# gkm2708/gym-lmaze

Measured on AMD Instinct MI355X. Metric: env steps/sec (whole node), 1M parallel 11x11 mazes at 1/2/4/8 MI355X, higher is better.
Workload: dtype int32

## Files before the change

gym-lmaze_amd/csrc/lmaze_step.hip:

```cpp
#include <cstdio>

#include <cmath>
#include <cstdlib>

#include "lmaze_common.h"
#include "lmaze_policy_table.h"

namespace lmaze {

static constexpr size_t kNonTemporalObsBytes = (size_t)192 << 20;

template <bool NT, int BITS = 0>
__device__ __forceinline__ void store16(int4* p, const int4& v) {
    typedef int v4i __attribute__((ext_vector_type(4)));
    if (NT) {
        v4i t = {v.x, v.y, v.z, v.w};
        stream_store16<BITS>(reinterpret_cast<v4i*>(p), t);
    } else {
        *p = v;
    }
}

__device__ __forceinline__ void count_goal(int32_t* p) { __hip_atomic_fetch_add(p, 1, __ATOMIC_RELAXED, __HIP_MEMORY_SCOPE_AGENT); }

__host__ __device__ inline bool beyond_caches(int64_t n, int cells) { return (size_t)n * cells * 4 > kNonTemporalObsBytes; }

struct EnvState {
    int2 b, g;
    int act, sc, done;
    float r;
};

template <int VARIANT, bool DO_STEP>
__device__ __forceinline__ EnvState load_env(const StepArgs& a, int64_t e) {
    constexpr bool V3 = VARIANT == LMAZE_VARIANT_V3;
    EnvState in;
    in.b = a.ball[e];
    in.g = make_int2(-1, -1);
    if (V3) in.g = a.goal[e];
    in.act = 0; in.sc = 0; in.done = 0; in.r = 0.0f;
    if (DO_STEP) {
        in.act = a.action[e];
        in.sc = a.step_count[e];
        if (!V3) in.r = a.reward[e];
        const uint8_t* dp = a.auto_reset ? a.done + e : a.layout;
        in.done = *dp;
    }
    return in;
}

template <int VARIANT>
__device__ __forceinline__ void env_reset(int ball_cell, int goal_cell, int G, EnvState& s) {
    if (ball_cell >= 0) s.b = make_int2(ball_cell / G, ball_cell % G);
    if (VARIANT == LMAZE_VARIANT_V3 && goal_cell >= 0) s.g = make_int2(goal_cell / G, goal_cell % G);
    s.sc = 0;
    s.r = -0.0f;
}

__device__ __forceinline__ void clamp_ball(EnvState& s, int G) { s.b = make_int2(clampi(s.b.x, 0, G - 1), clampi(s.b.y, 0, G - 1)); }

template <int VARIANT, class CellAt>
__device__ __forceinline__ bool env_advance(const StepArgs& a, int G, CellAt cell_at, EnvState& s) {
    int bx = clampi(s.b.x, 0, G - 1), by = clampi(s.b.y, 0, G - 1);
    s.sc += 1;
    int ox, oy;
    decode_action(s.act, ox, oy);
    const int tx = clampi(bx + ox, 0, G - 1), ty = clampi(by + oy, 0, G - 1);
    float r;
    bool dn;
    const bool hit = transition_rule<VARIANT>(a, cell_at(tx, ty), ox, oy, tx, ty, s.sc, s.r, s.g.x, s.g.y, bx, by, r, dn);
    s.b = make_int2(bx, by);
    s.r = r;
    s.done = dn ? 1 : 0;
    return hit;
}

__device__ __forceinline__ void store_state(const StepArgs& a, int64_t e, const EnvState& s) {
    a.ball[e] = s.b;
    a.step_count[e] = s.sc;
    a.reward[e] = s.r;
    a.done[e] = s.done;
}

__device__ __forceinline__ int ball_cell_of(const int2& b, int G) { return b.x * G + b.y; }
template <int VARIANT>
__device__ __forceinline__ int goal_cell_of(const int2& g, int G) {
// ... 427 lines not shown
                a.step_count[e] = sc;
                a.reward[e] = r;
                a.done[e] = dn ? 1 : 0;
            }
            b = make_int2(bx, by);
        } else {
            b = make_int2(clampi(b.x, 0, G - 1), clampi(b.y, 0, G - 1));
        }
        if (a.obs == nullptr) continue;
        const int bcell = b.x * G + b.y;
        const int gcell = (V3 && g.x >= 0 && g.x < G && g.y >= 0 && g.y < G) ? g.x * G + g.y : -8;
        int4* obs4 = reinterpret_cast<int4*>(a.obs + (size_t)e * CELLS);
#pragma unroll
        for (int j = 0; j < NJ; ++j) {
            const int c0 = (j * 64 + lane) << 2;
            int vals[4];
#pragma unroll
            for (int q = 0; q < 4; ++q) {
                int v = cell_bits<VARIANT>((uint8_t)(w[j] >> (8 * q)));
                v |= (bcell == c0 + q) ? LMAZE_OBS_BALL : 0;
                if (V3) v |= (gcell == c0 + q) ? LMAZE_OBS_GOAL : 0;
                vals[q] = v;
            }
            store16<NT, 2>(obs4 + j * 64 + lane, make_int4(vals[0], vals[1], vals[2], vals[3]));
        }
    }
}


template <int VARIANT, bool DO_STEP, int EPW>
__global__ __launch_bounds__(LMAZE_BLOCK) void step_shared_wave8_kernel(const StepArgs a) {
    constexpr bool V3 = VARIANT == LMAZE_VARIANT_V3;
    constexpr int G = 8, CELLS = 64;
    const int lane = threadIdx.x & 63;
    const int64_t base = ((int64_t)blockIdx.x * (blockDim.x >> 6) + (threadIdx.x >> 6)) * EPW;
    if (base >= a.n) return;
    const int nb = (int)min((int64_t)EPW, a.n - base);
    const bool autoreset = DO_STEP && a.auto_reset;
    const uint64_t epoch = step_epoch(a, autoreset);
    const bool live = lane < nb;
    const int myc = a.layout[lane];
    EnvState s{};
    s.b = make_int2(1, 1); s.g = make_int2(-1, -1);
    if (live) s = load_env<VARIANT, DO_STEP>(a, base + lane);
    const int mypat = cell_bits<VARIANT>((uint8_t)myc);
    const int p4 = (lane & 15) << 2;
    const int4 pat4 = make_int4(__shfl(mypat, p4, 64), __shfl(mypat, p4 + 1, 64), __shfl(mypat, p4 + 2, 64),
                                __shfl(mypat, p4 + 3, 64));
    int4* obs4 = reinterpret_cast<int4*>(a.obs + (size_t)base * CELLS);
    if (DO_STEP) {
        if (autoreset) {
            const unsigned long long ok[1] = {__ballot(interior(lane, G) && spawn_ok<VARIANT>((uint8_t)myc))};
            if (s.done) {
                int bc, gc;
                place_from_masks<VARIANT, 1>(ok, __popcll(ok[0]), env_draw(a.seed, epoch, a.env_base + base + lane), bc, gc);
                env_reset<VARIANT>(bc, gc, G, s);
                if (V3 && gc >= 0 && live) a.goal_rw[base + lane] = s.g;
            }
        }
        const bool hit = env_advance<VARIANT>(a, G, [&](int tx, int ty) { return (uint8_t)__shfl(myc, tx * G + ty, 64); }, s);
        if (live) {
            const int64_t e = base + lane;
            if (hit && a.goal_count) count_goal(a.goal_count + e);
            store_state(a, e, s);
        }
    } else {
        clamp_ball(s, G);
    }
    if (a.obs == nullptr) return;
    const int ball_cell = ball_cell_of(s.b, G);
    const int goal_cell = goal_cell_of<VARIANT>(s.g, G);
#pragma unroll
    for (int k = 0; k < EPW / 4; ++k) {
        const int le = (lane >> 4) + 4 * k;
        const int bc = __shfl(ball_cell, le, 64);
        const int gc = V3 ? __shfl(goal_cell, le, 64) : -8;
        int4 v = pat4;
        or_at(v, bc - p4, LMAZE_OBS_BALL);
        if (V3) or_at(v, gc - p4, LMAZE_OBS_GOAL);
        if (le < nb) obs4[lane + 64 * k] = v;
    }
}

template <int VARIANT, bool DO_STEP, int EPB>
__global__ __launch_bounds__(LMAZE_BLOCK) void step_shared_u8_kernel(const StepArgs a) {
    constexpr bool V3 = VARIANT == LMAZE_VARIANT_V3;
    static_assert(EPB % 16 == 0 && EPB <= LMAZE_BLOCK, "a workgroup's byte range starts on a 16-byte boundary; one lane per env");
    const int G = a.grid, CELLS = G * G;
    const int PW = (2 * CELLS + 16 + 3) >> 2;
    extern __shared__ int4 lds4[];
    uint32_t* patw = reinterpret_cast<uint32_t*>(lds4);
    int* ballflat = reinterpret_cast<int*>(patw + 4 * PW);
    int* goalflat = ballflat + EPB + 1;
    int* maskflag = goalflat + EPB + 1;
    uint16_t* spawn = reinterpret_cast<uint16_t*>(maskflag + EPB + 1);
    uint8_t* lay = reinterpret_cast<uint8_t*>(spawn + ((CELLS + 1) & ~1));
    __shared__ int spawn_count_s;
    const int tid = threadIdx.x;
    const int64_t nchunks = (a.n + EPB - 1) / EPB;
    int64_t chunk = blockIdx.x;
    int64_t blockbase = chunk * EPB;
    int nb = (int)min((int64_t)EPB, a.n - blockbase);
    const bool masked = !DO_STEP && a.mask != nullptr;
    const bool autoreset = DO_STEP && a.auto_reset;
    const uint64_t epoch = step_epoch(a, autoreset);
    EnvState in{};
    if (tid < nb) in = load_env<VARIANT, DO_STEP>(a, blockbase + tid);
    int warmed = 0;
    if (DO_STEP && (a.launch_hint & 0x100)) {
        warmed = warm_lines(a.action, a.n * 4, 256) + warm_lines(a.ball, a.n * 8, 256) + warm_lines(a.step_count, a.n * 4, 256);
        if (!V3) warmed += warm_lines(a.reward, a.n * 4, 256);
        if (V3) warmed += warm_lines(a.goal, a.n * 8, 256);
        if (autoreset) warmed += warm_lines(a.done, a.n, 256);
    }
    for (int i = tid; i < CELLS; i += LMAZE_BLOCK) lay[i] = a.layout[i];
    __syncthreads();
    uint8_t* patb = reinterpret_cast<uint8_t*>(patw);
    for (int i = tid; i < 4 * PW; i += LMAZE_BLOCK) {
        const int s = i / PW, k = (i - s * PW) << 2;
        uint32_t w = 0;
#pragma unroll
        for (int j = 0; j < 4; ++j) {
            int c = k + s + j;
            c -= c >= CELLS ? CELLS : 0;
            c -= c >= CELLS ? CELLS : 0;
            c = min(c, CELLS - 1);
            w |= (uint32_t)cell_bits<VARIANT>(lay[c]) << (8 * j);
        }
        patw[i] = w;
    }
    if (autoreset && tid < 64) {
        const int cnt = wave_build_spawn_list<VARIANT>(lay, G, CELLS, spawn, tid);
        if (tid == 0) spawn_count_s = cnt;
    }
    if (tid == 0) { ballflat[EPB] = -64; goalflat[EPB] = -64; maskflag[EPB] = 0; }
    __syncthreads();
  for (;;) {
    const int64_t next = chunk + gridDim.x;
    const bool has_next = next < nchunks;
    EnvState in_next{};
    int nb_next = 0;
    if (has_next) {
        nb_next = (int)min((int64_t)EPB, a.n - next * EPB);
        if (tid < nb_next) in_next = load_env<VARIANT, DO_STEP>(a, next * EPB + tid);
    }
    if (tid < EPB) {
        int bf = -64, gf = -64, mf = 0;
        if (tid < nb) {
            const int64_t e = blockbase + tid;
            int bc, gc;
            const int cnt = autoreset ? spawn_count_s : 0;
            env_phase1<VARIANT, DO_STEP>(a, lay, G, e, in, [&](uint4 d, int& pb, int& pg) { place_from_list<VARIANT>(spawn, cnt, d, pb, pg); }, epoch, bc, gc);
            bf = bc;
            if (V3 && gc >= 0) gf = gc;
            if (masked) mf = a.mask[e] != 0;
        }
        ballflat[tid] = bf;
        goalflat[tid] = gf;
        maskflag[tid] = mf;
    }
    if (a.obs8 != nullptr) {
    __syncthreads();
    uint8_t* obs = a.obs8 + (size_t)blockbase * CELLS;
    const int R = nb * CELLS;
    if (!masked) {
        const int nq = R >> 4;
        for (int q = tid; q < nq; q += LMAZE_BLOCK) {
// ... 528 lines not shown
    if (layout_mode != LMAZE_LAYOUT_SHARED) return launch_perenv<GT, VARIANT, DO_STEP>(a, s);
    if constexpr (GT == 8) {
        const bool small = a.obs == nullptr || !beyond_caches(a.n, 64);
        if (small && a.mask == nullptr && (a.launch_hint & 0x100) == 0) {
            int code = (a.launch_hint >> 4) & 15;
            if (code < 1 || code > 3) code = a.n >= 65536 ? 1 : 2;
            const int epw = 128 >> code;
            int wpb = a.launch_hint & 15;
            if (wpb != 1 && wpb != 2 && wpb != 4) wpb = a.n >= 65536 ? 4 : 1;
            const int64_t waves = (a.n + epw - 1) / epw;
            const int64_t blocks = (waves + wpb - 1) / wpb;
            if (!grid_ok(blocks)) return hipErrorInvalidConfiguration;
            const dim3 grid((unsigned)blocks), block(64 * wpb);
            if (a.info) {
                char name[96];
                snprintf(name, sizeof(name), "step_shared_wave8_kernel<v%d, %s, %d>", VARIANT, DO_STEP ? "step" : "observe", epw);
                describe_launch(a.info, name, epw * wpb, 0, 1, false, blocks, 64 * wpb, 0);
                return hipSuccess;
            }
            if (code == 1) hipLaunchKernelGGL((step_shared_wave8_kernel<VARIANT, DO_STEP, 64>), grid, block, 0, s, a);
            else if (code == 2) hipLaunchKernelGGL((step_shared_wave8_kernel<VARIANT, DO_STEP, 32>), grid, block, 0, s, a);
            else hipLaunchKernelGGL((step_shared_wave8_kernel<VARIANT, DO_STEP, 16>), grid, block, 0, s, a);
            return hipGetLastError();
        }
        int sel = (a.launch_hint >> 10) & 3;
        if (sel == 0) sel = table_sel<VARIANT>(a, a.obs != nullptr ? 2 : 1);
        if (sel == 2) return launch_shared<GT, VARIANT, DO_STEP, 64>(a, s);
        return launch_shared<GT, VARIANT, DO_STEP, 128>(a, s);
    } else if constexpr (GT == 11 || GT == 12) {
        int sel = (a.launch_hint >> 10) & 3;
        const bool streaming = a.obs != nullptr && beyond_caches(a.n, GT * GT);
        if (sel == 0) {
            if (GT == 11) sel = streaming ? 2 : 1;
            else sel = streaming ? 3 : 1;
            if (streaming) sel = table_sel<VARIANT>(a, sel);
        }
        if (sel == 2) return launch_shared<GT, VARIANT, DO_STEP, 32>(a, s);
        if (sel == 3) return launch_shared<GT, VARIANT, DO_STEP, 16>(a, s);
        return launch_shared<GT, VARIANT, DO_STEP, 64>(a, s);
    } else if constexpr (GT == 14 || GT == 18) {
        int sel = (a.launch_hint >> 10) & 3;
        const bool streaming = a.obs != nullptr && beyond_caches(a.n, GT * GT);
        if (sel == 0) sel = ((GT == 14 || VARIANT == LMAZE_VARIANT_V3) && streaming) ? 2 : 1;
        if (((a.launch_hint >> 10) & 3) == 0 && streaming) sel = table_sel<VARIANT>(a, sel);
        if (sel == 2) return launch_shared<GT, VARIANT, DO_STEP, 16>(a, s);
        return launch_shared<GT, VARIANT, DO_STEP, 32>(a, s);
    } else if constexpr (GT == 32) {
        int sel = (a.launch_hint >> 10) & 3;
        const bool streaming = a.obs != nullptr && beyond_caches(a.n, GT * GT);
        if (sel == 0) sel = streaming ? table_sel<VARIANT>(a, 2) : 1;
        if (sel == 2) return launch_shared<GT, VARIANT, DO_STEP, 4>(a, s);
        return launch_shared<GT, VARIANT, DO_STEP, 8>(a, s);
    } else {
        int sel = (a.launch_hint >> 10) & 3;
        if (sel == 0) {
            sel = a.grid >= 15 ? 3 : (a.grid >= 5 ? 2 : 1);
            if (a.obs != nullptr && beyond_caches(a.n, a.grid * a.grid) && a.grid >= 5) sel = table_sel<VARIANT>(a, sel);
        }
        if (sel == 3) return launch_shared<GT, VARIANT, DO_STEP, 16>(a, s);
        if (sel == 2) return launch_shared<GT, VARIANT, DO_STEP, 64>(a, s);
        return launch_shared<GT, VARIANT, DO_STEP, 256>(a, s);
    }
}

template <int VARIANT, bool DO_STEP>
static hipError_t dispatch_grid(const StepArgs& a, int layout_mode, hipStream_t s) {
    switch (a.grid) {
        case 8:  return launch_one<8, VARIANT, DO_STEP>(a, layout_mode, s);
        case 11: return launch_one<11, VARIANT, DO_STEP>(a, layout_mode, s);
        case 12: return launch_one<12, VARIANT, DO_STEP>(a, layout_mode, s);
        case 14: return launch_one<14, VARIANT, DO_STEP>(a, layout_mode, s);
        case 18: return launch_one<18, VARIANT, DO_STEP>(a, layout_mode, s);
        case 32: return launch_one<32, VARIANT, DO_STEP>(a, layout_mode, s);
        default: return launch_one<0, VARIANT, DO_STEP>(a, layout_mode, s);
    }
}

hipError_t launch_step(int variant, bool do_step, const StepArgs& a, int layout_mode, hipStream_t s);

#ifndef LMAZE_U8_DEFAULT_SEL
#define LMAZE_U8_DEFAULT_SEL 1
#endif
#ifndef LMAZE_U8_DEFAULT_CHUNKS
#define LMAZE_U8_DEFAULT_CHUNKS 2
#endif
template <int EPB>
static hipError_t launch_step_u8_epb(int variant, bool do_step, const StepArgs& a, hipStream_t s) {
    const int cells = a.grid * a.grid, pw = (2 * cells + 16 + 3) >> 2;
    const size_t lds = ((size_t)4 * pw * 4 + 3 * (size_t)(EPB + 1) * 4 + (size_t)((cells + 1) & ~1) * 2 + (size_t)cells + 15) & ~(size_t)15;
    int m = (a.launch_hint >> 4) & 15;
    if (m == 0) m = LMAZE_U8_DEFAULT_CHUNKS;
    const int64_t nchunks = (a.n + EPB - 1) / EPB;
    const int64_t blocks = (nchunks + m - 1) / m;
    if (!grid_ok(blocks)) return hipErrorInvalidConfiguration;
    if (a.info) {
        char name[96];
        snprintf(name, sizeof(name), "step_shared_u8_kernel<v%d, %s, %d>", variant, do_step ? "step" : "observe", EPB);
        describe_launch(a.info, name, EPB, 0, m, false, blocks, LMAZE_BLOCK, lds);
        return hipSuccess;
    }
    const dim3 grid((unsigned)blocks), block(LMAZE_BLOCK);
    StepArgs b = a;
    b.launch_hint = (a.launch_hint & ~0x100) | ((size_t)a.n * cells > ((size_t)64 << 20) ? 0x100 : 0);
    if (variant == LMAZE_VARIANT_V3) {
        if (do_step) hipLaunchKernelGGL((step_shared_u8_kernel<LMAZE_VARIANT_V3, true, EPB>), grid, block, lds, s, b);
        else hipLaunchKernelGGL((step_shared_u8_kernel<LMAZE_VARIANT_V3, false, EPB>), grid, block, lds, s, b);
    } else {
        if (do_step) hipLaunchKernelGGL((step_shared_u8_kernel<LMAZE_VARIANT_V0, true, EPB>), grid, block, lds, s, b);
        else hipLaunchKernelGGL((step_shared_u8_kernel<LMAZE_VARIANT_V0, false, EPB>), grid, block, lds, s, b);
    }
    return hipGetLastError();
}

hipError_t launch_step_u8(int variant, bool do_step, const StepArgs& a, hipStream_t s) {
    if (a.n == 0) return hipSuccess;
    int sel = (a.launch_hint >> 10) & 3;
    if (sel == 0) sel = LMAZE_U8_DEFAULT_SEL;
    if (sel == 1) return launch_step_u8_epb<256>(variant, do_step, a, s);
    if (sel == 2) return launch_step_u8_epb<128>(variant, do_step, a, s);
    return launch_step_u8_epb<64>(variant, do_step, a, s);
}

static bool slot_stores_nt(const StepArgs& a, const RolloutRec* rec) {
    return rec && rec->obs_t && ((a.launch_hint >> 15) & 1);
}

enum RolloutFamily { RO_WAVE8, RO_SHARED, RO_PERENV, RO_U8, RO_STEPS };
static const char* const kRolloutKernel[] = {"rollout_shared_wave8_kernel", "rollout_shared_kernel", "rollout_perenv_kernel",
                                             "rollout_shared_u8_kernel"};
struct RolloutPlan {
    RolloutFamily family;
    int epb;
    int block;
    int64_t blocks;
    size_t lds;
    bool nt;
};

static size_t rollout_u8_lds_bytes(int G, int epb) {
    const int cells = G * G, pw = (2 * cells + 16 + 3) >> 2;
    return ((size_t)4 * pw * 4 + 2 * (size_t)(epb + 1) * 4 + (size_t)((cells + 1) & ~1) * 2 + (size_t)cells + 15) & ~(size_t)15;
}

static size_t policy_table_lds_bytes(int G) { return (size_t)((G * G + 15) & ~15); }

enum { PLAN_OPEN = 0, PLAN_POLICY = 1, PLAN_SAMPLE_LDS = 2, PLAN_SAMPLE_GLOBAL = 3 };
static RolloutPlan rollout_plan(const StepArgs& a, int layout_mode, int32_t T, const RolloutRec* rec, bool u8, int pol = PLAN_OPEN) {
    const int cells = a.grid * a.grid;
    const bool sample = pol == PLAN_SAMPLE_LDS || pol == PLAN_SAMPLE_GLOBAL;
    const size_t tab = pol == PLAN_POLICY ? policy_table_lds_bytes(a.grid) : pol == PLAN_SAMPLE_LDS ? (size_t)16 * cells : 0;
    const int hint_epb = (a.launch_hint >> 12) & 7;
    const bool planes = a.obs != nullptr || (rec && rec->obs_t);
    RolloutPlan p{RO_STEPS, 0, LMAZE_BLOCK, 0, 0, false};
    if (u8) {
        int epb = a.n >= 65536 ? 64 : 16;
        if (rec && rec->obs_t && a.n >= 262144) epb = 256;
        if (hint_epb) epb = 4 << (hint_epb - 1);
        if (epb < 16) epb = 16;
        if (epb > LMAZE_BLOCK) epb = LMAZE_BLOCK;
        while (epb > 16 && rollout_u8_lds_bytes(a.grid, epb) + tab > ((size_t)64 << 10)) epb >>= 1;
        p.family = RO_U8;
        p.epb = epb;
        p.lds = rollout_u8_lds_bytes(a.grid, epb) + tab;
    } else if (!pol && layout_mode == LMAZE_LAYOUT_SHARED && a.grid == 8 && (!planes || !beyond_caches(a.n, 64)) &&
               (a.launch_hint & 0x100) == 0) {
        p.family = RO_WAVE8;
        p.block = 64 * (a.n >= 65536 ? 4 : 1);
        p.epb = p.block;
    } else if (pol || (T > 1 && (a.launch_hint & 0x100) == 0)) {
        const bool perenv = layout_mode == LMAZE_LAYOUT_PER_ENV;
        p.family = perenv ? RO_PERENV : RO_SHARED;
        int epb = a.n >= 65536 ? 64 : (a.n >= 16384 ? 32 : 16);
        if (perenv)
            while (epb > 4 && (size_t)epb * cells > (size_t)32 << 10) epb >>= 1;
        if (!rec && beyond_caches(a.n, cells))
            while (epb > 8 && (size_t)epb * cells * 4 > 12288) epb >>= 1;
        if (perenv && rec && epb == 32 && a.n < 65536) epb = 16;
        if (hint_epb) epb = 4 << (hint_epb - 1);
        if (perenv && epb > 64) epb = 64;
        auto lds_of = [&](int k) {
            const size_t own = perenv ? 2 * (size_t)k * 4 + (((size_t)k * cells + 15) & ~(size_t)15)
                                      : (size_t)cells * 4 + 2 * (size_t)k * 4 + (size_t)((cells + 15) & ~15) + (size_t)((cells * 2 + 15) & ~15);
            return tab + (sample ? (own + 15) & ~(size_t)15 : own);
        };
        if (perenv)
            while (epb > 4 && lds_of(epb) > (size_t)160 * 1024) epb >>= 1;
        p.epb = epb;
        p.lds = lds_of(epb);
        p.nt = slot_stores_nt(a, rec);
    }
    if (p.family != RO_STEPS) p.blocks = (a.n + p.epb - 1) / p.epb;
    return p;
}

template <class F>
static const void* kernel_of(int variant, F v3, F v0) { return (const void*)(variant == LMAZE_VARIANT_V3 ? v3 : v0); }

static const void* rollout_kernel(RolloutFamily f, int variant, bool rec) {
    using P = void (*)(const StepArgs, const RolloutArgs);
    using R = void (*)(const StepArgs, const RolloutObsArgs);
    using R8 = void (*)(const StepArgs, const RolloutObs8Args);
    constexpr int V0 = LMAZE_VARIANT_V0, V3 = LMAZE_VARIANT_V3;
    switch (f) {
// ... 125 lines not shown
```

include/lmaze.h:

```cpp
#ifndef LMAZE_H_
#define LMAZE_H_

#include <stdint.h>

#ifdef __cplusplus
extern "C" {
#endif

#define LMAZE_ABI_VERSION 4

enum {
    LMAZE_VARIANT_V0 = 0,
    LMAZE_VARIANT_V3 = 3
};

enum {
    LMAZE_LAYOUT_SHARED = 0,
    LMAZE_LAYOUT_PER_ENV = 1
};

enum {
    LMAZE_OBS_BALL = 1,
    LMAZE_OBS_WALL = 2,
    LMAZE_OBS_GOAL = 4,
    LMAZE_OBS_FREE = 8
};

enum {
    LMAZE_E_NULL = -1,
    LMAZE_E_GRID = -2,
    LMAZE_E_VARIANT = -3,
    LMAZE_E_LAYOUT = -4,
    LMAZE_E_COUNT = -5,
    LMAZE_E_ALIGN = -6,
    LMAZE_E_EXPANSION = -7,
    LMAZE_E_NODEVICE = -8
};

#define LMAZE_MAX_GRID 64
#define LMAZE_MAX_ENVS ((int64_t)1 << 30)
#define LMAZE_MAX_CHANNELS 8

typedef struct LmazeParams {
    int32_t variant;
    int32_t grid;
    int32_t layout_mode;
    int32_t step_limit;
    float reward_wall;
    float reward_move;
    float reward_goal;
    int32_t launch_hint;
} LmazeParams;

int lmaze_abi_version(void);

const char* lmaze_strerror(int code);

int lmaze_device_info(int device, int32_t* cu_count_host, char* name_host, int32_t name_len);

int lmaze_describe_step(const LmazeParams* params, int64_t n, int32_t auto_reset, int32_t with_obs, char* text_host,
                        int32_t len);

int lmaze_step_v0(const LmazeParams* params, const uint8_t* layout, const int32_t* action,
                  int32_t* ball_xy, int32_t* step_count, float* reward, uint8_t* done,
                  int32_t* goal_count, int32_t* obs, int64_t n, void* stream);

int lmaze_step_v3(const LmazeParams* params, const uint8_t* layout, const int32_t* action,
                  int32_t* ball_xy, const int32_t* goal_xy, int32_t* step_count, float* reward,
                  uint8_t* done, int32_t* obs, int64_t n, void* stream);

int lmaze_observe(const LmazeParams* params, const uint8_t* layout, const int32_t* ball_xy,
                  const int32_t* goal_xy, int32_t* obs, int64_t n, void* stream);

int lmaze_reset(const LmazeParams* params, const uint8_t* layout, const uint8_t* mask,
                uint64_t seed, uint64_t epoch, int64_t env_base, int32_t* ball_xy, int32_t* goal_xy,
                int32_t* step_count, float* reward, uint8_t* done, int32_t* obs, int64_t n,
                void* stream);

int lmaze_step_v0_autoreset(const LmazeParams* params, const uint8_t* layout, const int32_t* action,
                            int32_t* ball_xy, int32_t* step_count, float* reward, uint8_t* done,
                            int32_t* goal_count, int32_t* obs, int64_t n, uint64_t seed,
                            uint64_t epoch, int64_t env_base, const uint64_t* epoch_in_dev,
                            uint64_t* epoch_out_dev, void* stream);

int lmaze_step_v3_autoreset(const LmazeParams* params, const uint8_t* layout, const int32_t* action,
                            int32_t* ball_xy, int32_t* goal_xy, int32_t* step_count, float* reward,
                            uint8_t* done, int32_t* obs, int64_t n, uint64_t seed, uint64_t epoch,
                            int64_t env_base, const uint64_t* epoch_in_dev, uint64_t* epoch_out_dev,
                            void* stream);

int lmaze_step_u8(const LmazeParams* params, const uint8_t* layout, const int32_t* action, int32_t* ball_xy, int32_t* goal_xy,
                  int32_t* step_count, float* reward, uint8_t* done, int32_t* goal_count, uint8_t* obs8, int64_t n,
                  int32_t auto_reset, uint64_t seed, uint64_t epoch, int64_t env_base, const uint64_t* epoch_in_dev,
                  uint64_t* epoch_out_dev, void* stream);
int lmaze_observe_u8(const LmazeParams* params, const uint8_t* layout, const int32_t* ball_xy, const int32_t* goal_xy,
                     const uint8_t* mask, uint8_t* obs8, int64_t n, void* stream);

int lmaze_rollout(const LmazeParams* params, const uint8_t* layout, const int32_t* actions, int32_t T, int32_t* ball_xy,
                  int32_t* goal_xy, int32_t* step_count, float* reward, uint8_t* done, int32_t* goal_count, int32_t* obs,
                  float* reward_t, uint8_t* done_t, int64_t n, int32_t auto_reset, uint64_t seed, uint64_t epoch,
                  int64_t env_base, void* stream);

int lmaze_rollout_obs(const LmazeParams* params, const uint8_t* layout, const int32_t* actions, int32_t T, int32_t* ball_xy,
                      int32_t* goal_xy, int32_t* step_count, float* reward, uint8_t* done, int32_t* goal_count, int32_t* obs,
                      float* reward_t, uint8_t* done_t, int64_t n, int32_t auto_reset, uint64_t seed, uint64_t epoch,
                      int64_t env_base, int32_t* obs_t, int32_t obs_every, void* stream);

int lmaze_rollout_u8(const LmazeParams* params, const uint8_t* layout, const int32_t* actions, int32_t T, int32_t* ball_xy,
                     int32_t* goal_xy, int32_t* step_count, float* reward, uint8_t* done, int32_t* goal_count, uint8_t* obs8,
                     float* reward_t, uint8_t* done_t, int64_t n, int32_t auto_reset, uint64_t seed, uint64_t epoch,
                     int64_t env_base, void* stream);

int lmaze_rollout_obs_u8(const LmazeParams* params, const uint8_t* layout, const int32_t* actions, int32_t T, int32_t* ball_xy,
                         int32_t* goal_xy, int32_t* step_count, float* reward, uint8_t* done, int32_t* goal_count, uint8_t* obs8,
                         float* reward_t, uint8_t* done_t, int64_t n, int32_t auto_reset, uint64_t seed, uint64_t epoch,
                         int64_t env_base, uint8_t* obs_t8, int32_t obs_every, void* stream);

int lmaze_describe_rollout(const LmazeParams* params, int64_t n, int32_t T, int32_t auto_reset, int32_t with_obs,
                           int32_t obs_every, char* text_host, int32_t len);

int lmaze_rollout_policy(const LmazeParams* params, const uint8_t* layout, const uint8_t* policy, int32_t key_mode,
                         uint32_t epsilon_u32, int32_t T, int32_t* ball_xy, int32_t* goal_xy, int32_t* step_count, float* reward,
                         uint8_t* done, int32_t* goal_count, int32_t* obs, float* reward_t, uint8_t* done_t, int32_t* actions_t,
                         int32_t* key_t, int64_t n, int32_t auto_reset, uint64_t seed, uint64_t epoch, int64_t env_base,
                         int32_t* obs_t, int32_t obs_every, void* stream);

int lmaze_rollout_policy_u8(const LmazeParams* params, const uint8_t* layout, const uint8_t* policy, int32_t key_mode,
                            uint32_t epsilon_u32, int32_t T, int32_t* ball_xy, int32_t* goal_xy, int32_t* step_count, float* reward,
                            uint8_t* done, int32_t* goal_count, uint8_t* obs8, float* reward_t, uint8_t* done_t, int32_t* actions_t,
                            int32_t* key_t, int64_t n, int32_t auto_reset, uint64_t seed, uint64_t epoch, int64_t env_base,
                            uint8_t* obs_t8, int32_t obs_every, void* stream);

int lmaze_describe_rollout_policy(const LmazeParams* params, int64_t n, int32_t T, int32_t auto_reset, int32_t with_obs,
                                  int32_t obs_every, int32_t key_mode, char* text_host, int32_t len);

int lmaze_rollout_sample(const LmazeParams* params, const uint8_t* layout, const uint32_t* thresholds, int32_t key_mode, int32_t T,
                         int32_t* ball_xy, int32_t* goal_xy, int32_t* step_count, float* reward, uint8_t* done, int32_t* goal_count,
                         int32_t* obs, float* reward_t, uint8_t* done_t, int32_t* actions_t, int32_t* key_t, int64_t n,
                         int32_t auto_reset, uint64_t seed, uint64_t epoch, int64_t env_base, int32_t* obs_t, int32_t obs_every,
                         void* stream);

int lmaze_rollout_sample_u8(const LmazeParams* params, const uint8_t* layout, const uint32_t* thresholds, int32_t key_mode, int32_t T,
                            int32_t* ball_xy, int32_t* goal_xy, int32_t* step_count, float* reward, uint8_t* done,
                            int32_t* goal_count, uint8_t* obs8, float* reward_t, uint8_t* done_t, int32_t* actions_t, int32_t* key_t,
                            int64_t n, int32_t auto_reset, uint64_t seed, uint64_t epoch, int64_t env_base, uint8_t* obs_t8,
                            int32_t obs_every, void* stream);

int lmaze_describe_rollout_sample(const LmazeParams* params, int64_t n, int32_t T, int32_t auto_reset, int32_t with_obs,
                                  int32_t obs_every, int32_t key_mode, char* text_host, int32_t len);

int lmaze_returns(const float* reward_t, const uint8_t* done_t, const float* tail, float gamma, float* returns_t, int32_t T,
                  int64_t n, void* stream);

int lmaze_render_expanded(const int32_t* obs, int32_t grid, int32_t expansion,
                          const int32_t* channel_mask_host, int32_t channels, float* out,
                          int64_t n, void* stream);

int lmaze_episode_stats(const uint8_t* done, const float* reward, const int32_t* step_count,
                        const int32_t* goal_count, float reward_goal, int64_t n, int64_t* out4, void* stream);

int lmaze_bandwidth_probe(const void* src, void* dst, int64_t bytes, void* stream);

enum {
    LMAZE_VARIANT_V1 = 1,
    LMAZE_VARIANT_V2 = 2,
    LMAZE_VARIANT_V4 = 4,
    LMAZE_VARIANT_V5 = 5,
    LMAZE_VARIANT_V6 = 6
};

#define LMAZE_FOVEA 5
#define LMAZE_MAX_LAYOUTS 16

// ... 96 lines not shown
```

Measured before the change: 13.66 billion.

## Add grid-specialized u8 step kernel with periodic 16-byte obs pattern

Adds a compile-time grid-size specialization of the u8 step kernel. The observation background is precomputed in LDS as a pattern whose period is lcm(cells,16) bytes, so each 16-byte store takes one pattern word and ORs in the ball and goal bits for at most two envs. This replaces the generic per-byte or per-word assembly. It also switches the default chunks-per-block to 1, adds an LDS padding cap that limits workgroups per CU for non-autoreset runs, sets waves_per_eu, and pipelines the next chunk's env load. The extra template instances add code size, and the occupancy cap could cost latency hiding.

```diff
diff --git a/gym-lmaze_amd/csrc/lmaze_step.hip b/gym-lmaze_amd/csrc/lmaze_step.hip
--- a/gym-lmaze_amd/csrc/lmaze_step.hip
+++ b/gym-lmaze_amd/csrc/lmaze_step.hip
@@ -2,6 +2,7 @@
 
 #include <cmath>
 #include <cstdlib>
+#include <type_traits>
 
 #include "lmaze_common.h"
 #include "lmaze_policy_table.h"
@@ -595,7 +596,170 @@
     }
 }
 
-template <int VARIANT, bool DO_STEP, int EPB>
+__device__ __forceinline__ void or_byte16(uint4& w, int b, uint32_t bit) {
+    const uint32_t m = (unsigned)b < 16u ? bit << ((b & 3) << 3) : 0u;
+    const int d = b >> 2;
+    w.x |= (d == 0) ? m : 0u;
+    w.y |= (d == 1) ? m : 0u;
+    w.z |= (d == 2) ? m : 0u;
+    w.w |= (d == 3) ? m : 0u;
+}
+
+template <int GT>
+struct U8Period {
+    static constexpr int CELLS = GT * GT;
+    static constexpr int GCD = CELLS % 16 == 0 ? 16 : (CELLS % 8 == 0 ? 8 : (CELLS % 4 == 0 ? 4 : (CELLS % 2 == 0 ? 2 : 1)));
+    static constexpr int GRP = 16 / GCD;
+    static constexpr int P = GRP * CELLS / 16;
+};
+
+template <int GT, int VARIANT, int EPB>
+__device__ __forceinline__ void step_u8_grid_body(const StepArgs& a) {
+    constexpr bool V3 = VARIANT == LMAZE_VARIANT_V3;
+    constexpr int G = GT, CELLS = GT * GT, GRP = U8Period<GT>::GRP, P = U8Period<GT>::P;
+    static_assert(EPB % GRP == 0, "a workgroup's byte range starts on a period boundary");
+    constexpr int NONE = -4096;
+    extern __shared__ int4 lds4[];
+    uint4* pat16 = reinterpret_cast<uint4*>(lds4);
+    uint8_t* patb = reinterpret_cast<uint8_t*>(pat16);
+    int* ballflat = reinterpret_cast<int*>(pat16 + P);
+    int* goalflat = ballflat + EPB + 1;
+    uint8_t* lay = reinterpret_cast<uint8_t*>(goalflat + EPB + 1);
+    const int tid = threadIdx.x;
+    const int64_t nchunks = (a.n + EPB - 1) / EPB;
+    int64_t chunk = blockIdx.x;
+    int64_t blockbase = chunk * EPB;
+    int nb = (int)min((int64_t)EPB, a.n - blockbase);
+    const bool autoreset = a.auto_reset;
+    const bool nt = (a.launch_hint & 0x100) != 0;
+    const uint64_t epoch = autoreset ? launch_epoch(a.epoch, a.epoch_in) : 0;
+    if (autoreset) pass_epoch_on(a.epoch_in, a.epoch_out);
+    EnvState in{};
+    if (tid < nb) in = load_env<VARIANT, true>(a, blockbase + tid);
+    if (nt && !autoreset && !(a.launch_hint & 0x200)) asm volatile("s_waitcnt vmcnt(0)" ::: "memory");
+    int warmed = 0;
+    if (nt) {
+        warmed = warm_lines(a.action, a.n * 4, 256) + warm_lines(a.ball, a.n * 8, 256) + warm_lines(a.step_count, a.n * 4, 256);
+        if (!V3) warmed += warm_lines(a.reward, a.n * 4, 256);
+        if (V3) warmed += warm_lines(a.goal, a.n * 8, 256);
+        if (autoreset) warmed += warm_lines(a.done, a.n, 256);
+    }
+    constexpr int NL = (CELLS + LMAZE_BLOCK - 1) / LMAZE_BLOCK, NS = (CELLS + 63) / 64;
+    unsigned long long okm[NS] = {};
+    int okcount = 0;
+    {
+        uint8_t cb[NL], sb[NS];
+#pragma unroll
+        for (int j = 0; j < NL; ++j) cb[j] = a.layout[min(tid + j * LMAZE_BLOCK, CELLS - 1)];
+        if (autoreset) {
+#pragma unroll
+            for (int j = 0; j < NS; ++j) sb[j] = a.layout[min((tid & 63) + j * 64, CELLS - 1)];
+        }
+#pragma unroll
+        for (int j = 0; j < NL; ++j) {
+            const int c = tid + j * LMAZE_BLOCK;
+            if (c < CELLS) {
+                lay[c] = cb[j];
+                const uint8_t bits = (uint8_t)cell_bits<VARIANT>(cb[j]);
+#pragma unroll
+                for (int g = 0; g < GRP; ++g) patb[g * CELLS + c] = bits;
+            }
+        }
+        if (autoreset) {
+#pragma unroll
+            for (int j = 0; j < NS; ++j) {
+                const int c = (tid & 63) + j * 64;
+                okm[j] = __ballot(c < CELLS && interior(c, G) && spawn_ok<VARIANT>(sb[j]));
+                okcount += __popcll(okm[j]);
+            }
+        }
+    }
+    if (tid == 0) { ballflat[EPB] = NONE; goalflat[EPB] = NONE; }
+    __syncthreads();
+  for (;;) {
+    const int64_t next = chunk + gridDim.x;
+    const bool has_next = next < nchunks;
+    EnvState in_next{};
+    int nb_next = 0;
+    if (has_next) {
+        nb_next = (int)min((int64_t)EPB, a.n - next * EPB);
+        if (tid < nb_next) in_next = load_env<VARIANT, true>(a, next * EPB + tid);
+    }
+    if (tid < EPB) {
+        int bf = NONE, gf = NONE;
+        if (tid < nb) {
+            int bc, gc;
+            env_phase1<VARIANT, true>(a, lay, G, blockbase + tid, in, [&](uint4 d, int& pb, int& pg) { place_from_masks<VARIANT, NS>(okm, okcount, d, pb, pg); }, epoch, bc, gc);
+            bf = bc;
+            if (V3 && gc >= 0) gf = gc;
+        }
+        ballflat[tid] = bf;
+        if (V3) goalflat[tid] = gf;
+    }
+    if (a.obs8 != nullptr) {
+    __syncthreads();
+    uint8_t* obs = a.obs8 + (size_t)blockbase * CELLS;
+    const int R = nb * CELLS, nq = R >> 4;
+    constexpr int U = V3 ? 2 : 4;
+    for (int q0 = tid; q0 < nq; q0 += U * LMAZE_BLOCK) {
+        uint4 w[U];
+        int c[U], b0[U], b1[U], g0[U], g1[U];
+#pragma unroll
+        for (int u = 0; u < U; ++u) {
+            const int q = min(q0 + u * LMAZE_BLOCK, nq - 1);
+            const int grp = q / P, p = q - grp * P;
+            const int li = GRP == 1 ? 0 : (p << 4) / CELLS;
+            const int le = grp * GRP + li;
+            c[u] = (p << 4) - li * CELLS;
+            w[u] = pat16[p];
+            b0[u] = ballflat[le];
+            b1[u] = GRP == 1 ? NONE : ballflat[le + 1];
+            g0[u] = V3 ? goalflat[le] : NONE;
+            g1[u] = (V3 && GRP != 1) ? goalflat[le + 1] : NONE;
+        }
+#pragma unroll
+        for (int u = 0; u < U; ++u) {
+            const int q = q0 + u * LMAZE_BLOCK;
+            if (q < nq) {
+                or_byte16(w[u], b0[u] - c[u], LMAZE_OBS_BALL);
+                if (GRP != 1) or_byte16(w[u], CELLS - c[u] + b1[u], LMAZE_OBS_BALL);
+                if (V3) {
+                    or_byte16(w[u], g0[u] - c[u], LMAZE_OBS_GOAL);
+                    if (GRP != 1) or_byte16(w[u], CELLS - c[u] + g1[u], LMAZE_OBS_GOAL);
+                }
+                if (nt) {
+                    typedef unsigned v4u __attribute__((ext_vector_type(4)));
+                    v4u t = {w[u].x, w[u].y, w[u].z, w[u].w};
+                    stream_store16(reinterpret_cast<v4u*>(obs) + q, t);
+                } else {
+                    reinterpret_cast<uint4*>(obs)[q] = w[u];
+                }
+            }
+        }
+    }
+    for (int f = (nq << 4) + tid; f < R; f += LMAZE_BLOCK) {
+        const int le = f / CELLS, cc = f - le * CELLS;
+        obs[f] = (uint8_t)(patb[cc] | (ballflat[le] == cc ? LMAZE_OBS_BALL : 0) | (V3 && goalflat[le] == cc ? LMAZE_OBS_GOAL : 0));
+    }
+    }
+    if (!has_next) break;
+    __syncthreads();
+    chunk = next;
+    blockbase = chunk * EPB;
+    nb = nb_next;
+    in = in_next;
+  }
+    if (warmed == 0x7fedcba9 && a.n < 0) a.done[0] = 1;
+}
+
+template <int GT, int VARIANT, bool DO_STEP, int EPB, std::enable_if_t<GT != 0, int> = 0>
+__global__ __launch_bounds__(LMAZE_BLOCK) __attribute__((amdgpu_waves_per_eu(8, 8))) void step_shared_u8_kernel(const StepArgs a) {
+    static_assert(DO_STEP, "the render-only launches keep the generic body");
+    static_assert(EPB % 16 == 0 && EPB <= LMAZE_BLOCK, "a workgroup's byte range starts on a 16-byte boundary; one lane per env");
+    step_u8_grid_body<GT, VARIANT, EPB>(a);
+}
+
+template <int GT, int VARIANT, bool DO_STEP, int EPB, std::enable_if_t<GT == 0, int> = 0>
 __global__ __launch_bounds__(LMAZE_BLOCK) void step_shared_u8_kernel(const StepArgs a) {
     constexpr bool V3 = VARIANT == LMAZE_VARIANT_V3;
     static_assert(EPB % 16 == 0 && EPB <= LMAZE_BLOCK, "a workgroup's byte range starts on a 16-byte boundary; one lane per env");
@@ -1290,43 +1454,90 @@
 #define LMAZE_U8_DEFAULT_SEL 1
 #endif
 #ifndef LMAZE_U8_DEFAULT_CHUNKS
-#define LMAZE_U8_DEFAULT_CHUNKS 2
+#define LMAZE_U8_DEFAULT_CHUNKS 1
 #endif
-template <int EPB>
+#ifndef LMAZE_U8_DEFAULT_CAP
+#define LMAZE_U8_DEFAULT_CAP(auto_reset) ((auto_reset) ? 0 : 6)
+#endif
+#ifndef LMAZE_U8_DEFAULT_STAGGER
+#define LMAZE_U8_DEFAULT_STAGGER 0
+#endif
+
+static size_t step_u8_lds_bytes(int G, int gt, int epb) {
+    const int cells = G * G;
+    if (gt != 0) {
+        const int gcd = cells % 16 == 0 ? 16 : (cells % 8 == 0 ? 8 : (cells % 4 == 0 ? 4 : (cells % 2 == 0 ? 2 : 1)));
+        return ((size_t)(16 / gcd) * cells + 2 * (size_t)(epb + 1) * 4 + (size_t)cells + 15) & ~(size_t)15;
+    }
+    const int pw = (2 * cells + 16 + 3) >> 2;
+    return ((size_t)4 * pw * 4 + 3 * (size_t)(epb + 1) * 4 + (size_t)((cells + 1) & ~1) * 2 + (size_t)cells + 15) & ~(size_t)15;
+}
+
+template <int GT, int EPB>
 static hipError_t launch_step_u8_epb(int variant, bool do_step, const StepArgs& a, hipStream_t s) {
-    const int cells = a.grid * a.grid, pw = (2 * cells + 16 + 3) >> 2;
-    const size_t lds = ((size_t)4 * pw * 4 + 3 * (size_t)(EPB + 1) * 4 + (size_t)((cells + 1) & ~1) * 2 + (size_t)cells + 15) & ~(size_t)15;
+    const int cells = a.grid * a.grid;
+    size_t lds = step_u8_lds_bytes(a.grid, GT, EPB);
+    const bool nt = (size_t)a.n * cells > ((size_t)64 << 20);
+    int per_cu = a.launch_hint & 15;
+    if (per_cu == 0) per_cu = LMAZE_U8_DEFAULT_CAP(a.auto_reset);
+    if (per_cu < 1 || per_cu >= 8) per_cu = 0;
+    if (per_cu) {
+        const size_t want = lds_for_workgroups_per_cu(per_cu);
+        if (want > lds) lds = want;
+    }
     int m = (a.launch_hint >> 4) & 15;
     if (m == 0) m = LMAZE_U8_DEFAULT_CHUNKS;
     const int64_t nchunks = (a.n + EPB - 1) / EPB;
     const int64_t blocks = (nchunks + m - 1) / m;
     if (!grid_ok(blocks)) return hipErrorInvalidConfiguration;
     if (a.info) {
-        char name[96];
-        snprintf(name, sizeof(name), "step_shared_u8_kernel<v%d, %s, %d>", variant, do_step ? "step" : "observe", EPB);
-        describe_launch(a.info, name, EPB, 0, m, false, blocks, LMAZE_BLOCK, lds);
+        char name[96], spec[16] = "";
+        if (GT != 0) snprintf(spec, sizeof(spec), " G=%d", GT);
+        snprintf(name, sizeof(name), "step_shared_u8_kernel<v%d, %s, %d>%s", variant, do_step ? "step" : "observe", EPB, spec);
+        describe_launch(a.info, name, EPB, per_cu, m, nt, blocks, LMAZE_BLOCK, lds);
         return hipSuccess;
     }
     const dim3 grid((unsigned)blocks), block(LMAZE_BLOCK);
     StepArgs b = a;
-    b.launch_hint = (a.launch_hint & ~0x100) | ((size_t)a.n * cells > ((size_t)64 << 20) ? 0x100 : 0);
-    if (variant == LMAZE_VARIANT_V3) {
-        if (do_step) hipLaunchKernelGGL((step_shared_u8_kernel<LMAZE_VARIANT_V3, true, EPB>), grid, block, lds, s, b);
-        else hipLaunchKernelGGL((step_shared_u8_kernel<LMAZE_VARIANT_V3, false, EPB>), grid, block, lds, s, b);
+    b.launch_hint = (a.launch_hint & ~0x100) | (nt ? 0x100 : 0);
+    if (!LMAZE_U8_DEFAULT_STAGGER) b.launch_hint |= 0x200;
+    constexpr int V0 = LMAZE_VARIANT_V0, V3 = LMAZE_VARIANT_V3;
+    if constexpr (GT != 0) {
+        if (variant == V3) hipLaunchKernelGGL((step_shared_u8_kernel<GT, V3, true, EPB>), grid, block, lds, s, b);
+        else hipLaunchKernelGGL((step_shared_u8_kernel<GT, V0, true, EPB>), grid, block, lds, s, b);
+    } else if (variant == V3) {
+        if (do_step) hipLaunchKernelGGL((step_shared_u8_kernel<0, V3, true, EPB>), grid, block, lds, s, b);
+        else hipLaunchKernelGGL((step_shared_u8_kernel<0, V3, false, EPB>), grid, block, lds, s, b);
     } else {
-        if (do_step) hipLaunchKernelGGL((step_shared_u8_kernel<LMAZE_VARIANT_V0, true, EPB>), grid, block, lds, s, b);
-        else hipLaunchKernelGGL((step_shared_u8_kernel<LMAZE_VARIANT_V0, false, EPB>), grid, block, lds, s, b);
+        if (do_step) hipLaunchKernelGGL((step_shared_u8_kernel<0, V0, true, EPB>), grid, block, lds, s, b);
+        else hipLaunchKernelGGL((step_shared_u8_kernel<0, V0, false, EPB>), grid, block, lds, s, b);
     }
     return hipGetLastError();
+}
+
+template <int EPB>
+static hipError_t launch_step_u8_grid(int variant, bool do_step, const StepArgs& a, hipStream_t s) {
+    if (do_step && !(a.launch_hint & LMAZE_HINT_U8_GENERIC)) {
+        switch (a.grid) {
+            case 8:  return launch_step_u8_epb<8, EPB>(variant, true, a, s);
+            case 11: return launch_step_u8_epb<11, EPB>(variant, true, a, s);
+            case 12: return launch_step_u8_epb<12, EPB>(variant, true, a, s);
+            case 14: return launch_step_u8_epb<14, EPB>(variant, true, a, s);
+            case 18: return launch_step_u8_epb<18, EPB>(variant, true, a, s);
+            case 32: return launch_step_u8_epb<32, EPB>(variant, true, a, s);
+            default: break;
+        }
+    }
+    return launch_step_u8_epb<0, EPB>(variant, do_step, a, s);
 }
 
 hipError_t launch_step_u8(int variant, bool do_step, const StepArgs& a, hipStream_t s) {
     if (a.n == 0) return hipSuccess;
     int sel = (a.launch_hint >> 10) & 3;
     if (sel == 0) sel = LMAZE_U8_DEFAULT_SEL;
-    if (sel == 1) return launch_step_u8_epb<256>(variant, do_step, a, s);
-    if (sel == 2) return launch_step_u8_epb<128>(variant, do_step, a, s);
-    return launch_step_u8_epb<64>(variant, do_step, a, s);
+    if (sel == 1) return launch_step_u8_grid<256>(variant, do_step, a, s);
+    if (sel == 2) return launch_step_u8_grid<128>(variant, do_step, a, s);
+    return launch_step_u8_grid<64>(variant, do_step, a, s);
 }
 
 static bool slot_stores_nt(const StepArgs& a, const RolloutRec* rec) {
diff --git a/include/lmaze.h b/include/lmaze.h
--- a/include/lmaze.h
+++ b/include/lmaze.h
@@ -89,6 +89,7 @@
                             int64_t env_base, const uint64_t* epoch_in_dev, uint64_t* epoch_out_dev,
                             void* stream);
 
+#define LMAZE_HINT_U8_GENERIC (1 << 16)
 int lmaze_step_u8(const LmazeParams* params, const uint8_t* layout, const int32_t* action, int32_t* ball_xy, int32_t* goal_xy,
                   int32_t* step_count, float* reward, uint8_t* done, int32_t* goal_count, uint8_t* obs8, int64_t n,
                   int32_t auto_reset, uint64_t seed, uint64_t epoch, int64_t env_base, const uint64_t* epoch_in_dev,
```

Measured after the change: 13.67 billion (median of 3 runs). Within noise of the previous version (+0.1%).
